# ai-decentralized/BloomBee

Hardware: AMD Instinct MI355X
Metric: decode tokens/sec, llama-3-8b greedy, pipeline over RCCL/xGMI (higher is better)
Workload: dtype bfloat16; 1 GPU; model=llama-3-8b, global_batch=32, seq_len=2048, parallelism=pp1, micro_batches=1

## Files before the change

bloombee_amd/models/llama/block.py:

```python
from __future__ import annotations

import math
from typing import Optional

import torch
import torch.nn.functional as F

from bloombee_amd import ops
from bloombee_amd.kv.paged import SessionHandle
from bloombee_amd.models.base import ModelConfig
from bloombee_amd.models.block_common import (
    FamilyBlock, RopeTables, pack_q4, paged_attention_qkv, rms_train,
    rope_attn_train, rotary_positions, split_heads, swiglu_mlp_train)


class LlamaBlock(FamilyBlock):
    def __init__(self, config: ModelConfig, layer_index: int = 0,
                 rope: Optional[RopeTables] = None):
        super().__init__(config, layer_index)
        H = config.hidden_size
        D = config.head_dim
        Hq, Hkv = config.num_attention_heads, config.num_key_value_heads
        I = config.intermediate_size
        self.Hq, self.Hkv, self.D, self.I = Hq, Hkv, D, I
        self.scale = 1.0 / math.sqrt(D)
        p = self.p
        self.input_norm_w = p(H)
        self.qkv_w = p((Hq + 2 * Hkv) * D, H)
        self.o_w = p(H, Hq * D)
        self.post_norm_w = p(H)
        self.gate_up_w = p(2 * I, H)
        self.down_w = p(H, I)
        self.rope = rope if rope is not None else RopeTables(config)
        self._ss_h2 = None
        self._ss_hidden = None
        self._ss_valid = False
        self._splitk_cnt = None

    def _fuse_norm_gate(self, hidden) -> bool:
        return (getattr(self, "_w4", None) is None
                and getattr(self, "lora_delta", None) is None
                and ops.fuse_norm_linear_ok(hidden, self.qkv_w)
                and self.I % 256 == 0 and (2 * self.I) % 64 == 0
                and (self.Hq * self.D) % 256 == 0
                and self.config.hidden_size % 64 == 0)

    def _ensure_ss_bufs(self, device) -> None:
        if self._ss_h2 is None or self._ss_h2.device != device:
            st = self.config.hidden_size // 64
            self._ss_h2 = torch.empty(st * 32, dtype=torch.float32,
                                      device=device)
            self._ss_hidden = torch.empty_like(self._ss_h2)
            self._splitk_cnt = torch.zeros(2 * st, dtype=torch.int32,
                                           device=device)

    @torch.no_grad()
    def fold_norm_weights(self):
        if getattr(self, "_norm_folded", False):
            return
        self._norm_fold_orig = (self.input_norm_w.detach().clone(),
                                self.post_norm_w.detach().clone())
        self.qkv_w.data = (self.qkv_w.float()
                           * self.input_norm_w.float()).to(self.qkv_w.dtype)
        self.gate_up_w.data = (self.gate_up_w.float()
                               * self.post_norm_w.float()).to(self.gate_up_w.dtype)
        self.input_norm_w.data.fill_(1.0)
        self.post_norm_w.data.fill_(1.0)
        self._norm_folded = True

    @torch.no_grad()
    def unfold_norm_weights(self):
        if not getattr(self, "_norm_folded", False):
            return
        inw, pnw = self._norm_fold_orig
        self.input_norm_w.data.copy_(inw)
        self.post_norm_w.data.copy_(pnw)
        den_i = inw.float().abs().clamp_min(1e-6) * inw.float().sign().where(
            inw.float() != 0, torch.ones_like(inw.float()))
        den_p = pnw.float().abs().clamp_min(1e-6) * pnw.float().sign().where(
            pnw.float() != 0, torch.ones_like(pnw.float()))
        self.qkv_w.data = (self.qkv_w.float() / den_i).to(self.qkv_w.dtype)
        self.gate_up_w.data = (self.gate_up_w.float() / den_p).to(self.gate_up_w.dtype)
        self._norm_folded = False

    @torch.no_grad()
    def quantize_weights_q4(self, keep_full: bool = False):
        pack_q4(self, ("qkv_w", "o_w", "gate_up_w", "down_w"), keep_full)
        return self

    def _lin(self, x, w, name, **kw):
        w4 = getattr(self, "_w4", None)
        if w4 is not None and name in w4:
            packed, scale, zero, N = w4[name]
            y = ops.linear_w4(x, packed, scale, zero, N, **kw)
        else:
            y = ops.linear(x, w, **kw)
        ld = getattr(self, "lora_delta", None)
        if ld is not None:
            d = ld(name, x)
            if d is not None:
                y = y + d
        return y

    def _post_qkv(self, qkv: torch.Tensor, B: int, T: int) -> torch.Tensor:
        return qkv

    def _post_qkv_train(self, q: torch.Tensor, k: torch.Tensor):
        return q, k

    @torch.no_grad()
    def forward_inference(
        self,
        hidden: torch.Tensor,
        kv: SessionHandle,
        start_pos: torch.Tensor,
        position_ids: Optional[torch.Tensor] = None,
        tree_mask: Optional[torch.Tensor] = None,
    ) -> torch.Tensor:
        B, T, H = hidden.shape
        Hq, Hkv, D = self.Hq, self.Hkv, self.D
        cfg = self.config

        fuse_norm = self._fuse_norm_gate(hidden)
        self._ss_valid = False
        if fuse_norm and not getattr(self, "_norm_folded", False):
            self.fold_norm_weights()
        pb = getattr(self, "prev_block", None)
        defer = (fuse_norm and type(self)._post_qkv is LlamaBlock._post_qkv
                 and ops.fuse_qkv_rope_ok(hidden, self.qkv_w, D))
        if fuse_norm and pb is not None and getattr(pb, "_ss_valid", False):
            qkv = ops.linear(hidden, self.qkv_w,
                             norm=(None, cfg.rms_norm_eps),
                             ss_in=pb._ss_hidden, defer_combine=defer)
        elif defer:
            x = ops.rms_norm(hidden, self.input_norm_w, cfg.rms_norm_eps)
            qkv = ops.linear(x, self.qkv_w, defer_combine=True)
        else:
            x = ops.rms_norm(hidden, self.input_norm_w, cfg.rms_norm_eps)
            qkv = self._lin(x, self.qkv_w, "qkv_w")
        if not defer:
            qkv = self._post_qkv(qkv, B, T)
        cos, sin = self.rope.get(hidden.device)
        kp = kv.k_pages(self.layer_index)
        vp = kv.v_pages(self.layer_index)
        pt = kv.page_table()
        position_ids = rotary_positions(kv, start_pos, position_ids, T)
        ctx_lens = None
        if defer and qkv.dtype == torch.float32:
            qkv, ctx_lens = ops.rope_kv_write_part(
                qkv, None, B, T, Hq, Hkv, cos, sin, position_ids, kp, vp, pt,
                start_pos)
        else:
            ops.rope_kv_write_(qkv, Hq, Hkv, cos, sin, position_ids, kp, vp,
                               pt, start_pos)
        attn = paged_attention_qkv(qkv, kv, self.layer_index, start_pos, Hq,
                                   Hkv, self.scale, tree_mask=tree_mask,
                                   ctx_lens=ctx_lens)
        if fuse_norm:
            self._ensure_ss_bufs(hidden.device)
            st = H // 64
            h2 = ops.linear(attn, self.o_w, residual=hidden,
                            ss_out=self._ss_h2,
                            cnt=(self._splitk_cnt[:st]
                                 if ops.inlaunch_combine_ok(attn, self.o_w, "o")
                                 else None))
            act = ops.linear_swiglu(h2, self.gate_up_w,
                                    norm=(None, cfg.rms_norm_eps),
                                    ss_in=self._ss_h2)
            out = ops.linear(act, self.down_w, residual=h2,
                             ss_out=self._ss_hidden,
                             cnt=(self._splitk_cnt[st:]
                                  if ops.inlaunch_combine_ok(act, self.down_w,
                                                             "down")
                                  else None))
            self._ss_valid = True
            return out
        a = self._lin(attn, self.o_w, "o_w")

        h2, y = ops.rms_norm_residual(a, hidden, self.post_norm_w, cfg.rms_norm_eps)
        return self._lin(ops.swiglu(self._lin(y, self.gate_up_w, "gate_up_w")),
                         self.down_w, "down_w", residual=h2)

    def forward_train(self, hidden: torch.Tensor, start_pos: int = 0) -> torch.Tensor:
        eps = self.config.rms_norm_eps

        def lin(x_, w, name):
            y = F.linear(x_, w)
            ld = getattr(self, "lora_delta", None)
            if ld is not None:
                d = ld(name, x_)
                if d is not None:
                    y = y + d
            return y

        x = rms_train(hidden, self.input_norm_w, eps)
        q, k, v = split_heads(lin(x, self.qkv_w, "qkv_w"), self.Hq, self.Hkv,
                              self.D)
        q, k = self._post_qkv_train(q, k)
        attn = rope_attn_train(q, k, v, self.rope, start_pos, self.scale)
        h2 = hidden + lin(attn, self.o_w, "o_w")
        y = rms_train(h2, self.post_norm_w, eps)
        return h2 + swiglu_mlp_train(y, self.gate_up_w, self.down_w)
```

bloombee_amd/ops/__init__.py:

```python
from bloombee_amd.ops.interface import (
    HAVE_HIP_OPS,
    alibi_slopes_for,
    attn_decode,
    attn_paged,
    attn_paged_mixed,
    attn_paged_mixed_qkv,
    attn_paged_qkv,
    attn_prefill,
    attn_train,
    fuse_norm_linear_ok,
    fuse_qkv_rope_ok,
    fuse_swiglu_ok,
    gelu_tanh,
    hip_ops,
    inlaunch_combine_ok,
    kv_gather,
    kv_write,
    layer_norm,
    linear,
    linear_swiglu,
    linear_w4,
    mfma_selftest,
    moe_gemm_grouped,
    moe_gemm_grouped_w4,
    quant4_pack,
    quant4_unpack,
    rms_norm,
    rms_norm_residual,
    rope_apply_,
    rope_kv_write_,
    rope_kv_write_part,
    rope_cos_sin,
    set_attn_sparsity,
    swiglu,
)
```

bloombee_amd/ops/hip/common.h:

```cpp
#pragma once

#include <hip/hip_runtime.h>

#define DEVINL __device__ __forceinline__

typedef __attribute__((ext_vector_type(8))) short short8;
typedef __attribute__((ext_vector_type(4))) short short4v;
typedef __attribute__((ext_vector_type(4))) float f32x4;
typedef __attribute__((ext_vector_type(2))) float f32x2;

static constexpr int WAVE = 64;
static constexpr float LOG2E = 1.4426950408889634f;
static constexpr float NEG_BIG = -1e30f;

typedef __attribute__((ext_vector_type(8))) __bf16 bf16x8;
DEVINL bf16x8 as_bf16x8(short8 s) { return __builtin_bit_cast(bf16x8, s); }

DEVINL float bf2f(unsigned short u) {
  union { unsigned int i; float f; } v;
  v.i = ((unsigned int)u) << 16;
  return v.f;
}

DEVINL unsigned short f2bf(float f) {
// ... 19 lines not shown
  *reinterpret_cast<short8*>(p) = v;
}

DEVINL float wave_reduce_sum(float x) {
#pragma unroll
  for (int m = 1; m < WAVE; m <<= 1) x += __shfl_xor(x, m);
  return x;
}

DEVINL float wave_reduce_max(float x) {
#pragma unroll
  for (int m = 1; m < WAVE; m <<= 1) x = fmaxf(x, __shfl_xor(x, m));
  return x;
}

DEVINL float group16_reduce_sum(float x) {
#pragma unroll
  for (int m = 1; m < 16; m <<= 1) x += __shfl_xor(x, m);
  return x;
}

DEVINL float group16_reduce_max(float x) {
#pragma unroll
  for (int m = 1; m < 16; m <<= 1) x = fmaxf(x, __shfl_xor(x, m));
  return x;
}

DEVINL float fast_exp2(float x) { return __builtin_amdgcn_exp2f(x); }

DEVINL float fast_expf(float x) { return __builtin_amdgcn_exp2f(x * LOG2E); }

DEVINL long ldiv_up(long a, long b) { return (a + b - 1) / b; }

#define HIP_OK(expr)                                                         \
  do {                                                                       \
    hipError_t _e = (expr);                                                  \
    if (_e != hipSuccess) {                                                  \
      TORCH_CHECK(false, "HIP error: ", hipGetErrorString(_e), " at ",       \
                  __FILE__, ":", __LINE__);                                  \
    }                                                                        \
  } while (0)
```

bloombee_amd/ops/hip/ext.hip:

```cpp

#include <torch/extension.h>
#include <c10/hip/HIPStream.h>
#include <hip/hip_runtime.h>
#include <cstdlib>

#include "common.h"

#include "elementwise.hip"
#include "kvcache.hip"
#include "attn_decode.hip"
#include "attn_decode_mfma.hip"
#include "attn_sparse.hip"
#include "attn_prefill.hip"
#include "attn_train.hip"
#include "gemm_skinny.hip"
#include "moe_gemm.hip"
#include "w4_gemm.hip"
#include "moe_gemm_w4.hip"
#include "mfma_selftest.hip"
#include "quant4.hip"
#include "wire.h"

typedef __attribute__((ext_vector_type(8))) short short8_h;

// ... 129 lines not shown
  int ksplit = (int)ksplit_req;
  if (ksplit <= 0) {
    static const int ks_big = [] {
      const char* e = std::getenv("BBAMD_GEMM_KSPLIT_BIG");
      return e ? std::atoi(e) : 1;
    }();
    if (N / 64 >= 256) ksplit = ks_big;
    else ksplit = (int)std::min<long>(K / 512,
                                      std::max<long>(1, std::min<long>(8, 1024 / (N / 64))));
    ksplit = std::max(1, ksplit);
  }
  if (K % 256 != 0)
    return {ksplit, (int)((K / 32 + ksplit - 1) / ksplit) * 32, false};
  const SplitK s = split_k_chunks((int)K, 256, ksplit);
  return {s.ksplit, s.kchunk, true};
}

static constexpr int kWringDepths[] = {2, 4};

static int skinny_wring(long req) {
  static const int env = [] {
    const char* e = std::getenv("BBAMD_GEMM_WRING");
    return e ? std::atoi(e) : 0;
  }();
  if (req <= 0) req = env;
  if (req <= 0) return 2;
  TORCH_CHECK(std::find(std::begin(kWringDepths), std::end(kWringDepths), req) !=
                  std::end(kWringDepths),
              "gemm_skinny W ring depth must be 2 or 4, got ", req);
  return (int)req;
}

template <int MT, int EPI, typename... Args>
static void launch_skinny_v2(int depth, dim3 grid, Args... args) {
  if (depth == 2)
    gemm_skinny_v2_kernel<MT, EPI><<<grid, 256, 0, cur_stream()>>>(args...);
  else
    gemm_skinny_v2_ring_kernel<MT, EPI, 4><<<grid, 256, 0, cur_stream()>>>(args...);
}

struct W4Plan {
  bool gemv;
  int ksplit, kchunk;
};

static W4Plan w4_plan(long M, long N, long K, long ksplit_req) {
  TORCH_CHECK(N >= 64 && K >= 128 && K % 128 == 0 && N % 64 == 0,
              "K%128, N%64 required");
  if (M == 1 && K % 2048 == 0 && K / 2048 <= 7) return {true, 1, (int)K};
  int ksplit = (int)ksplit_req;
  if (ksplit <= 0) {
    ksplit = (int)std::max<long>(1, std::min<long>(K / 512, 1792 / (N / 64)));
  }
  const SplitK s = split_k_chunks((int)K, 128, ksplit);
  return {false, s.ksplit, s.kchunk};
}

static SplitK moe_w4_plan(long E, long N, long K, long S, long ksplit_req) {
  TORCH_CHECK(N >= 64 && K >= 128 && K % 128 == 0 && N % 64 == 0,
              "K%128, N%64 required");
  int ksplit = (int)ksplit_req;
  if (ksplit <= 0) {
    const long blocks = (N / 64) * std::max<long>(1, std::min<long>(E, S));
    ksplit = (int)std::max<long>(1, std::min<long>(K / 512, 1792 / blocks));
  }
  return split_k_chunks((int)K, 128, ksplit);
}
// ... 836 lines not shown
  dim3 grid(N / 64, ksplit);
  dispatch_mtile(M, [&](auto mt) {
    gemm_skinny_w4_kernel<decltype(mt)::value><<<grid, 256, 0, cur_stream()>>>(
        ap, qp, scp, zp, ksplit == 1 ? rp : nullptr, ksplit == 1 ? bp : nullptr,
        cp, part.p, M, N, K, plan.kchunk, ksplit);
  });
  if (ksplit > 1) {
    const long total = (long)M * N;
    const int cgrid = (int)std::min<long>((total + 255) / 256, 2048);
    gemm_skinny_combine_kernel<<<cgrid, 256, 0, cur_stream()>>>(
        part.p, rp, bp, cp, M, N, ksplit);
  }
  return C;
}


static const float* ss_in_operand(const Operands& ops,
                                  const c10::optional<torch::Tensor>& ss_in,
                                  int* nstripes) {
  *nstripes = 0;
  if (!ss_in.has_value()) return nullptr;
  TORCH_CHECK(ss_in->numel() % 32 == 0, "ss_in must be f32 (nstripes,32)");
  *nstripes = (int)(ss_in->numel() / 32);
  return ops.ptr<F32>(*ss_in, "ss_in");
}

torch::Tensor gemm_skinny(torch::Tensor A, torch::Tensor W,
                          c10::optional<torch::Tensor> residual,
                          c10::optional<torch::Tensor> bias, long ksplit_req,
                          c10::optional<torch::Tensor> norm_w, double eps,
                          c10::optional<torch::Tensor> ss_in,
                          c10::optional<torch::Tensor> ss_out,
                          long norm_mode_req, bool defer_combine,
                          c10::optional<torch::Tensor> cnt, long wring_req) {
  Operands ops(A, "A");
  const auto* ap = ops.ptr<Bf16>(A, "A");
  const auto* wp = ops.ptr<Bf16>(W, "W");
  const int K = A.size(-1);
  const int M = A.numel() / K;
  const int N = W.size(0);
  TORCH_CHECK(M <= 32, "gemm_skinny is for M <= 32, got ", M);
  TORCH_CHECK(W.size(1) == K, "A/W K mismatch");
  TORCH_CHECK(K % 32 == 0 && N % 64 == 0, "K%32, N%64 required");
  int norm_mode = (int)norm_mode_req;
  const auto* nwp = ops.ptr<Bf16>(norm_w, "norm_w", true, K);
  if (nwp && norm_mode == 0) norm_mode = 1;
  TORCH_CHECK(norm_mode != 1 || nwp, "norm_mode 1 needs norm_w");
  if (norm_mode)
    TORCH_CHECK(K % 256 == 0, "fused rmsnorm needs the v2 (K%256) kernel");
  TORCH_CHECK(!ss_in.has_value() || norm_mode != 0,
              "ss_in only meaningful with a norm mode");
  int nstripes = 0;
  const float* ssinp = ss_in_operand(ops, ss_in, &nstripes);
  float* ssoutp = ops.ptr<F32>(ss_out, "ss_out", true, (long)(N / 64) * 32);
  const auto* rp = ops.ptr<Bf16>(residual, "residual", true, (long)M * N);
  const auto* bp = ops.ptr<Bf16>(bias, "bias", true, N);
  int* cntp = ops.ptr<I32>(cnt, "cnt");
  auto sizes = A.sizes().vec();
  sizes.back() = N;
  auto C = torch::empty(sizes, A.options());
  auto* cp = ops.ptr<Bf16>(C, "C");
  const SkinnyPlan plan = skinny_plan(N, K, ksplit_req);
  const int ksplit = plan.ksplit, kchunk = plan.kchunk;
  const Slabs part = alloc_slabs(ops, A, ksplit, M, N);
  const int wring =
      !plan.v2 ? 0
      : norm_mode == 1
          ? 2
          : skinny_wring(wring_req);
  if (cnt.has_value() && ksplit > 1 && plan.v2) {
    TORCH_CHECK(!defer_combine, "cnt and defer_combine exclude each other");
    TORCH_CHECK(cnt->numel() >= N / 64, "cnt must be int32 of >= N/64 entries");
    dispatch_mtile(M, [&](auto mt) {
      launch_skinny_v2<decltype(mt)::value, 2>(
          wring, dim3((N / 64) * ksplit), ap, wp, rp, bp, cp, part.p, M, N, K,
          kchunk, ksplit, nwp, (float)eps, norm_mode, ssinp, nstripes, ssoutp,
          cntp);
    });
    return C;
  }
  dim3 grid(N / 64, ksplit);
  dispatch_mtile(M, [&](auto mt) {
    if (plan.v2)
      launch_skinny_v2<decltype(mt)::value, 0>(
          wring, grid, ap, wp, ksplit == 1 ? rp : nullptr,
          ksplit == 1 ? bp : nullptr, cp, part.p, M, N, K, kchunk, ksplit, nwp,
          (float)eps, norm_mode, ssinp, nstripes,
          ksplit == 1 ? ssoutp : nullptr, (int*)nullptr);
    else {
      TORCH_CHECK(!norm_mode && (!ssoutp || ksplit > 1),
                  "fused norm / ss_out need the v2 (K%256) kernel");
      gemm_skinny_kernel<decltype(mt)::value><<<grid, 256, 0, cur_stream()>>>(
          ap, wp, ksplit == 1 ? rp : nullptr, ksplit == 1 ? bp : nullptr, cp,
          part.p, M, N, K, ksplit);
    }
  });
  if (ksplit > 1 && defer_combine) {
    TORCH_CHECK(!rp && !ssoutp, "defer_combine takes no residual / ss_out");
    return part.t;
  }
  if (ksplit > 1) {
    if (ssoutp || (N % 64 == 0 && N / 64 >= 64)) {
      dim3 cg(N / 64, (M + 15) / 16);
      gemm_skinny_combine_ss_kernel<<<cg, 256, 0, cur_stream()>>>(
          part.p, rp, bp, cp, ssoutp, M, N, ksplit);
    } else {
      const long total = (long)M * N;
      const int cgrid = (int)std::min<long>((total + 255) / 256, 2048);
      gemm_skinny_combine_kernel<<<cgrid, 256, 0, cur_stream()>>>(
          part.p, rp, bp, cp, M, N, ksplit);
    }
  }
  return C;
}

torch::Tensor gemm_skinny_swiglu(torch::Tensor A, torch::Tensor W, double eps,
                                 c10::optional<torch::Tensor> ss_in,
                                 long norm_mode_req, long wring_req) {
  Operands ops(A, "A");
  const auto* ap = ops.ptr<Bf16>(A, "A");
  const auto* wp = ops.ptr<Bf16>(W, "W");
  const int K = A.size(-1);
  const int M = A.numel() / K;
  const int N = W.size(0);
  const int I = N / 2;
  const int norm_mode = (int)norm_mode_req;
  TORCH_CHECK(M >= 1 && M <= 32, "gemm_skinny_swiglu is for 1 <= M <= 32, got ", M);
  TORCH_CHECK(W.dim() == 2 && W.size(1) == K, "A/W K mismatch");
  TORCH_CHECK(N % 2 == 0 && I % 32 == 0 && K % 256 == 0,
              "gemm_skinny_swiglu needs I % 32 == 0 and K % 256 == 0");
  TORCH_CHECK(norm_mode == 0 || norm_mode == 2, "norm_mode must be 0 or 2");
  TORCH_CHECK(!ss_in.has_value() || norm_mode == 2,
              "ss_in only meaningful with norm_mode 2");
  int nstripes = 0;
  const float* ssinp = ss_in_operand(ops, ss_in, &nstripes);
  auto sizes = A.sizes().vec();
  sizes.back() = I;
  auto C = torch::empty(sizes, A.options());
  auto* cp = ops.ptr<Bf16>(C, "C");
  const int wring = skinny_wring(wring_req);
  dispatch_mtile(M, [&](auto mt) {
    launch_skinny_v2<decltype(mt)::value, 1>(
        wring, dim3(I / 32), ap, wp, (const unsigned short*)nullptr,
        (const unsigned short*)nullptr, cp, (float*)nullptr, M, N, K, K, 1,
        (const unsigned short*)nullptr, (float)eps, norm_mode, ssinp, nstripes,
        (float*)nullptr, (int*)nullptr);
  });
  return C;
}


std::vector<torch::Tensor> quant4_pack(torch::Tensor x) {
  Operands ops(x, "x");
  const auto* xp = ops.ptr<Bf16>(x, "x");
  const long ncols = x.size(-1);
  TORCH_CHECK(ncols % 64 == 0, "quant4 needs cols % 64 == 0");
  const long nrows = x.numel() / ncols;
  auto packed = torch::empty({nrows, ncols / 2}, x.options().dtype(at::kByte));
  auto scale = torch::empty({nrows, ncols / 64}, x.options().dtype(at::kHalf));
  auto zero = torch::empty_like(scale);
  const long ngroups = nrows * (ncols / 64);
  if (ngroups == 0) return {packed, scale, zero};
  const int wpb = 4;
  quant4_pack_kernel<64><<<(ngroups + wpb - 1) / wpb, wpb * 64, 0, cur_stream()>>>(
      xp, ops.ptr<U8>(packed, "packed"), ops.ptr<F16>(scale, "scale"),
      ops.ptr<F16>(zero, "zero"), nrows, ncols);
  return {packed, scale, zero};
}

torch::Tensor quant4_unpack(torch::Tensor packed, torch::Tensor scale,
                            torch::Tensor zero) {
  Operands ops(packed, "packed");
  auto* qp = ops.ptr<U8>(packed, "packed");
  TORCH_CHECK(packed.dim() == 2, "packed must be (rows, cols/2)");
  const long nrows = packed.size(0), ncols = packed.size(1) * 2;
  TORCH_CHECK(ncols % 64 == 0, "quant4 needs cols % 64 == 0");
// ... 38 lines not shown
  return C;
}

PYBIND11_MODULE(TORCH_EXTENSION_NAME, m) {
  m.def("rms_norm", &rms_norm);
  m.def("rms_norm_residual", &rms_norm_residual);
  m.def("layer_norm", &layer_norm);
  m.def("rope_apply_", &rope_apply_);
  m.def("swiglu", &swiglu);
  m.def("gelu_tanh", &gelu_tanh);
  m.def("add_bf16", &add_bf16);
  m.def("kv_write", &kv_write);
  m.def("kv_gather", &kv_gather);
  m.def("wire_deflate", &wire_deflate);
  m.def("wire_inflate", &wire_inflate);
  m.def("wire_deflate_mt", &wire_deflate_mt);
  m.def("wire_inflate_mt", &wire_inflate_mt);
  m.def("attn_decode", &attn_decode);
  m.def("attn_decode_qkv", &attn_decode_qkv);
  m.def("attn_decode_mixed", &attn_decode_mixed);
  m.def("attn_decode_sparse", &attn_decode_sparse);
  m.def("attn_decode_sparse_qkv", &attn_decode_sparse_qkv);
  m.def("attn_prefill_qkv", &attn_prefill_qkv);
  m.def("rope_kv_write_", &rope_kv_write_);
  m.def("attn_prefill", &attn_prefill);
  m.def("attn_train_fwd", &attn_train_fwd);
  m.def("attn_train_bwd", &attn_train_bwd);
  m.def("gemm_skinny", &gemm_skinny, py::arg("A"), py::arg("W"),
        py::arg("residual") = c10::nullopt, py::arg("bias") = c10::nullopt,
        py::arg("ksplit") = 0, py::arg("norm_w") = c10::nullopt,
        py::arg("eps") = 0.0, py::arg("ss_in") = c10::nullopt,
        py::arg("ss_out") = c10::nullopt, py::arg("norm_mode") = 0,
        py::arg("defer_combine") = false, py::arg("cnt") = c10::nullopt,
        py::arg("wring") = 0);
  m.def("gemm_skinny_swiglu", &gemm_skinny_swiglu, py::arg("A"), py::arg("W"),
        py::arg("eps") = 0.0, py::arg("ss_in") = c10::nullopt,
        py::arg("norm_mode") = 0, py::arg("wring") = 0);
  m.def("gemm_skinny_plan", &gemm_skinny_plan);
  m.def("gemm_skinny_wring_plan", &gemm_skinny_wring_plan, py::arg("N"),
        py::arg("K"), py::arg("ksplit") = 0, py::arg("wring") = 0);
  m.def("rope_kv_write_part", &rope_kv_write_part);
  m.def("moe_gemm", &moe_gemm);
  m.def("gemm_w4", &gemm_w4);
  m.def("gemm_w4_plan", &gemm_w4_plan);
  m.def("moe_gemm_w4", &moe_gemm_w4);
  m.def("moe_gemm_w4_plan", &moe_gemm_w4_plan);
  m.def("quant4_pack", &quant4_pack);
  m.def("quant4_unpack", &quant4_unpack);
  m.def("mfma_selftest", &mfma_selftest);
  m.def("kv_stream_probe", &kv_stream_probe);
}
```

bloombee_amd/ops/hip/gemm_skinny.hip:

```cpp

#include "common.h"

template <int MT>
__global__ __launch_bounds__(256) void gemm_skinny_kernel(
    const unsigned short* __restrict__ A,
    const unsigned short* __restrict__ W,
    const unsigned short* __restrict__ R,
    const unsigned short* __restrict__ bias,
    unsigned short* __restrict__ C,
    float* __restrict__ Cpart,
    int M, int N, int K, int ksplit) {
  const int wave = threadIdx.x / WAVE;
  const int lane = threadIdx.x & (WAVE - 1);
  const int li = lane & 15;
  const int hi = lane >> 4;
  const int n0 = blockIdx.x * 64 + wave * 16;
  if (n0 >= N) return;
  const int split = blockIdx.y;
  const int kchunk = ((K / 32 + ksplit - 1) / ksplit) * 32;
  const int k0 = split * kchunk;
  const int k1 = min(K, k0 + kchunk);

  const unsigned short* wrow = W + (long)(n0 + li) * K;
  int arow[MT];
// ... 71 lines not shown
#pragma unroll
    for (int e = 0; e < 4; ++e) v[e] += p[e];
  }
#pragma unroll
  for (int e = 0; e < 4; ++e) {
    if (bias) v[e] += bf2f(bias[n0 + c4 + e]);
    if (R) v[e] += bf2f(R[i + e]);
  }
  short4v o4;
#pragma unroll
  for (int e = 0; e < 4; ++e) o4[e] = (short)f2bf(v[e]);
  *reinterpret_cast<short4v*>(C + i) = o4;
  if (ssout) {
    float vs = v[0] * v[0] + v[1] * v[1] + v[2] * v[2] + v[3] * v[3];
#pragma unroll
    for (int msk = 1; msk < 16; msk <<= 1) vs += __shfl_xor(vs, msk);
    if ((lane & 15) == 0) ssout[(long)stripe * 32 + m] = vs;
  }
}

template <int I>
struct WringIdx {
  static constexpr int value = I;
};

template <int DEPTH, int N, typename F>
DEVINL void wring_tail_dispatch(int nrem, F& f) {
  if constexpr (N <= 2 * DEPTH - 2) {
    if (nrem == N) f(WringIdx<N>{});
    else wring_tail_dispatch<DEPTH, N + 2>(nrem, f);
  }
}

template <int MT, int EPI, int DEPTH>
DEVINL void gemm_skinny_v2_body(
    const unsigned short* __restrict__ A,
    const unsigned short* __restrict__ W,
    const unsigned short* __restrict__ R,
    const unsigned short* __restrict__ bias,
    unsigned short* __restrict__ C,
    float* __restrict__ Cpart,
    int M, int N, int K, int kchunk, int ksplit,
    const unsigned short* __restrict__ nw,
    float eps, int norm_mode,
    const float* __restrict__ ssin,
    int nstripes,
    float* __restrict__ ssout,
    int* cnt) {
  static_assert(DEPTH == 2 || DEPTH % 4 == 0, "ring: whole waves per A row");
  constexpr int U = 4;
  constexpr int KSTEP = DEPTH * 128;
  constexpr int RSTRIDE = KSTEP + 8;
  constexpr int RPIECE = KSTEP / 8;
  constexpr int NPIECE = (32 * KSTEP) / (256 * 8);
  __shared__ __attribute__((aligned(16))) unsigned short atile[32 * RSTRIDE];
  __shared__ float ssp[256];
  __shared__ float invr[32];

  const int wave = threadIdx.x / WAVE;
  const int lane = threadIdx.x & (WAVE - 1);
  const int li = lane & 15;
  const int hi = lane >> 4;
  int tile = blockIdx.x;
  {
    const int nwg = gridDim.x;
    const int xcd = tile % 8, orig8 = tile / 8;
    const int q = nwg / 8, r = nwg % 8;
    if (nwg >= 8)
      tile = (xcd < r ? xcd * (q + 1) : r * (q + 1) + (xcd - r) * q) + orig8;
  }
  int split = blockIdx.y;
  if constexpr (EPI == 2) {
    split = tile % ksplit;
    tile /= ksplit;
  }
  const int n0 = tile * 64 + wave * 16;
  const int k0 = split * kchunk;
  const int k1 = min(K, k0 + kchunk);

  const unsigned short* wrow = W + (long)(n0 + li) * K;
  if constexpr (EPI == 1)
    wrow = W + ((long)(li < 8 ? 0 : N / 2 - 8) + tile * 32 + wave * 8 + li) * K;

  f32x4 acc[MT];
#pragma unroll
  for (int t = 0; t < MT; ++t) acc[t] = (f32x4){0.f, 0.f, 0.f, 0.f};

  short8 aregs[NPIECE];
  short8 nregs[DEPTH == 2 ? NPIECE : 1];
  const int wave_s = __builtin_amdgcn_readfirstlane(wave);
  auto load_a = [&](int ks, int lim = 1 << 30) {
#pragma unroll
    for (int j = 0; j < NPIECE; ++j) {
      if constexpr (DEPTH == 2) {
        const int flat = threadIdx.x + j * 256;
        const int row = min(flat / RPIECE, M - 1);
        const int off = (flat % RPIECE) * 8;
        aregs[j] = *reinterpret_cast<const short8*>(A + (long)row * K + ks + off);
        if (norm_mode == 1)
          nregs[j] = *reinterpret_cast<const short8*>(nw + ks + off);
      } else {
        const int fw = wave_s + j * 4;
        const int row = min(fw / (RPIECE / 64), M - 1);
        const unsigned off =
            min((fw % (RPIECE / 64)) * 64 + lane, lim / 8 - 1) * 16u;
        aregs[j] = *reinterpret_cast<const short8*>(
            reinterpret_cast<const char*>(A + (long)row * K + ks) + off);
      }
    }
  };
  auto store_a = [&]() {
#pragma unroll
    for (int j = 0; j < NPIECE; ++j) {
      const int flat = threadIdx.x + j * 256;
      short8 v = aregs[j];
      if (DEPTH == 2 && norm_mode == 1) {
        const float ir = invr[flat / RPIECE >= M ? M - 1 : flat / RPIECE];
#pragma unroll
        for (int e = 0; e < 8; ++e)
          v[e] = (short)f2bf(bf2f((unsigned short)v[e]) * ir *
                             bf2f((unsigned short)nregs[j][e]));
      }
      *reinterpret_cast<short8*>(atile + (flat / RPIECE) * RSTRIDE +
                                 (flat % RPIECE) * 8) = v;
    }
  };

  bf16x8 bB0[U], bB1[U];
  auto issue0 = [&](int k) {
#pragma unroll
    for (int u = 0; u < U; ++u)
      bB0[u] = as_bf16x8(
          *reinterpret_cast<const short8*>(wrow + k + u * 32 + hi * 8));
  };
  auto issue1 = [&](int k) {
#pragma unroll
    for (int u = 0; u < U; ++u)
      bB1[u] = as_bf16x8(
          *reinterpret_cast<const short8*>(wrow + k + u * 32 + hi * 8));
  };
  auto mfma_set = [&](bf16x8* bB, int half) {
#pragma unroll
    for (int u = 0; u < U; ++u)
#pragma unroll
      for (int t = 0; t < MT; ++t) {
        bf16x8 afrag = as_bf16x8(*reinterpret_cast<const short8*>(
            atile + (t * 16 + li) * RSTRIDE + half * 128 + u * 32 + hi * 8));
        acc[t] = __builtin_amdgcn_mfma_f32_16x16x32_bf16(afrag, bB[u], acc[t],
                                                         0, 0, 0);
      }
  };

  auto reduce_invr = [&]() {
    if (ssin) {
      const int row = threadIdx.x & 31, grp = threadIdx.x >> 5;
      float s0 = 0.f, s1 = 0.f, s2 = 0.f, s3 = 0.f;
      int s = grp;
      for (; s + 24 < nstripes; s += 32) {
        s0 += ssin[(long)s * 32 + row];
        s1 += ssin[(long)(s + 8) * 32 + row];
        s2 += ssin[(long)(s + 16) * 32 + row];
        s3 += ssin[(long)(s + 24) * 32 + row];
      }
      for (; s < nstripes; s += 8) s0 += ssin[(long)s * 32 + row];
      ssp[threadIdx.x] = (s0 + s1) + (s2 + s3);
      __syncthreads();
      if (threadIdx.x < 32) {
        float t = 0.f;
#pragma unroll
        for (int g = 0; g < 8; ++g) t += ssp[g * 32 + threadIdx.x];
        invr[threadIdx.x] = rsqrtf(t / K + eps);
      }
// ... 223 lines not shown
      __syncthreads();
      if (threadIdx.x < 32)
        ssout[(long)tile * 32 + threadIdx.x] =
            ssp[threadIdx.x] + ssp[32 + threadIdx.x] +
            ssp[64 + threadIdx.x] + ssp[96 + threadIdx.x];
    }
  } else {
    float* dst = Cpart + (long)split * M * N;
#pragma unroll
    for (int t = 0; t < MT; ++t)
#pragma unroll
      for (int reg = 0; reg < 4; ++reg) {
        const int m = t * 16 + hi * 4 + reg;
        if (m >= M) continue;
        float v = acc[t][reg];
        if (norm_mode == 2) v *= invr[m];
        dst[(long)m * N + n0 + li] = v;
      }
  }
}

#define SKINNY_V2_PARAMS                                                      \
  const unsigned short *__restrict__ A, const unsigned short *__restrict__ W, \
      const unsigned short *__restrict__ R,                                   \
      const unsigned short *__restrict__ bias, unsigned short *__restrict__ C, \
      float *__restrict__ Cpart, int M, int N, int K, int kchunk, int ksplit, \
      const unsigned short *__restrict__ nw, float eps, int norm_mode,        \
      const float *__restrict__ ssin, int nstripes, float *__restrict__ ssout, \
      int *cnt
#define SKINNY_V2_ARGS                                                       \
  A, W, R, bias, C, Cpart, M, N, K, kchunk, ksplit, nw, eps, norm_mode, ssin, \
      nstripes, ssout, cnt

template <int MT, int EPI = 0>
__global__ __launch_bounds__(256) void gemm_skinny_v2_kernel(SKINNY_V2_PARAMS) {
  gemm_skinny_v2_body<MT, EPI, 2>(SKINNY_V2_ARGS);
}

template <int MT, int EPI, int DEPTH>
__global__ __launch_bounds__(256, 3) void gemm_skinny_v2_ring_kernel(
    SKINNY_V2_PARAMS) {
  gemm_skinny_v2_body<MT, EPI, DEPTH>(SKINNY_V2_ARGS);
}

__global__ __launch_bounds__(256) void gemm_skinny_combine_ss_kernel(
    const float* __restrict__ Cpart, const unsigned short* __restrict__ R,
    const unsigned short* __restrict__ bias, unsigned short* __restrict__ C,
    float* __restrict__ ssout, int M, int N, int ksplit) {
  const int lane = threadIdx.x & (WAVE - 1);
  const int m = blockIdx.y * 16 + (threadIdx.x >> 6) * 4 + (lane >> 4);
  if (m >= M) return;
  gemm_skinny_combine_lane(Cpart, R, bias, C, ssout, M, N, ksplit, blockIdx.x,
                           m, lane);
}

__global__ void gemm_skinny_combine_kernel(
    const float* __restrict__ Cpart, const unsigned short* __restrict__ R,
    const unsigned short* __restrict__ bias, unsigned short* __restrict__ C,
    int M, int N, int ksplit) {
  const long total = (long)M * N;
  for (long i = blockIdx.x * (long)blockDim.x + threadIdx.x; i < total;
       i += (long)gridDim.x * blockDim.x) {
    float v = 0.f;
    for (int s = 0; s < ksplit; ++s) v += Cpart[(long)s * total + i];
    if (bias) v += bf2f(bias[i % N]);
    if (R) v += bf2f(R[i]);
    C[i] = f2bf(v);
  }
}
// ... 1 lines not shown
```

bloombee_amd/ops/interface.py:

```python
from __future__ import annotations

import importlib
import math
import os
from typing import Optional, Tuple

import torch

from bloombee_amd.ops import reference as ref
from bloombee_amd.ops.reference import alibi_slopes as alibi_slopes_for
from bloombee_amd.ops.reference import rope_cos_sin
from bloombee_amd.utils.logging import get_logger

logger = get_logger(__name__)

try:
    hip_ops = importlib.import_module("bloombee_amd.ops._hip_ops")
    HAVE_HIP_OPS = True
except ImportError as e:
    hip_ops = None
    HAVE_HIP_OPS = False
    _import_error = e


# ... 229 lines not shown
    if alibi_slopes is not None and not _on_gpu(q) and not sparse_decode:
        if scale is None:
            scale = 1.0 / math.sqrt(q.shape[-1])
        return ref.attn_paged(q, k_pages, v_pages, page_table, q_start, scale,
                              alibi_slopes=alibi_slopes,
                              sliding_window=_window_or_none(window))
    if tree_mask is not None:
        if scale is None:
            scale = 1.0 / math.sqrt(q.shape[-1])
        if (_on_gpu(q) and _TREE_KERNEL and window == 0
                and q.shape[-1] <= 256 and alibi_slopes is None):
            _require_ext()
            tm = tree_mask.to(q.device).contiguous().bool()
            return hip_ops.attn_prefill(q.contiguous(), k_pages, v_pages,
                                        page_table, q_start.int(), scale, 0,
                                        None, tm)
        return ref.attn_paged(q, k_pages, v_pages, page_table,
                              q_start.to(q.device), scale,
                              tree_mask=tree_mask.to(q.device))
    if Tq == 1:
        ctx_lens = q_start + 1
        return attn_decode(q, k_pages, v_pages, page_table, ctx_lens, scale,
                           window, alibi_slopes=alibi_slopes)
    return attn_prefill(q, k_pages, v_pages, page_table, q_start, scale, window,
                        alibi_slopes=alibi_slopes)


def linear(x: torch.Tensor, w: torch.Tensor, residual: Optional[torch.Tensor] = None,
           bias: Optional[torch.Tensor] = None,
           norm: Optional[tuple] = None,
           ss_in: Optional[torch.Tensor] = None,
           ss_out: Optional[torch.Tensor] = None,
           defer_combine: bool = False,
           cnt: Optional[torch.Tensor] = None) -> torch.Tensor:
    M = x.numel() // x.shape[-1]
    N, K = w.shape[0], x.shape[-1]
    if (_on_gpu(x) and M <= 32 and x.dtype == torch.bfloat16
            and K % 256 == 0 and N % 64 == 0):
        _require_ext()
        nw, eps, mode = None, 0.0, 0
        if norm is not None:
            eps = float(norm[1])
            if norm[0] is None:
                mode = 2
            else:
                nw = norm[0].contiguous()
                mode = 1
        return hip_ops.gemm_skinny(x.contiguous(), w, residual, bias,
                                   _INLAUNCH_KSPLIT if cnt is not None else 0,
                                   nw, eps, ss_in if norm is not None else None,
                                   ss_out, mode, defer_combine, cnt)
    if defer_combine or cnt is not None:
        raise RuntimeError("defer_combine / cnt require the GPU skinny-GEMM "
                           "path (callers gate on fuse_norm_linear_ok)")
    if norm is not None:
        nw = norm[0]
        if nw is None:
            nw = torch.ones(x.shape[-1], dtype=x.dtype, device=x.device)
        x = rms_norm(x, nw, norm[1])
    y = torch.nn.functional.linear(x, w, bias)
    if residual is not None:
        y = y + residual.view_as(y)
    if ss_out is not None:
        raise RuntimeError("ss_out requires the GPU skinny-GEMM path "
                           "(callers gate on fuse_norm_linear_ok)")
    return y


_FUSE_NORM = os.environ.get("BBAMD_FUSE_NORM", "1") != "0"


def fuse_norm_linear_ok(x: torch.Tensor, w: torch.Tensor) -> bool:
    K = x.shape[-1]
    return (_FUSE_NORM and _on_gpu(x) and x.numel() // K <= 32
            and x.dtype == torch.bfloat16 and K % 256 == 0
            and w.shape[0] % 64 == 0 and HAVE_HIP_OPS)


_FUSE_SWIGLU = os.environ.get("BBAMD_FUSE_SWIGLU", "1") != "0"
_FUSE_QKV_ROPE = os.environ.get("BBAMD_FUSE_QKV_ROPE", "1") != "0"
_INLAUNCH_DEFAULT = "0"


def _parse_inlaunch(v: str) -> frozenset:
    if v in ("", "0"):
        return frozenset()
    if v == "1":
        return frozenset(("o", "down"))
    return frozenset(x.strip() for x in v.split(",")) & {"o", "down"}


_INLAUNCH_COMBINE = _parse_inlaunch(
    os.environ.get("BBAMD_INLAUNCH_COMBINE", _INLAUNCH_DEFAULT))
_INLAUNCH_KSPLIT = int(os.environ.get("BBAMD_INLAUNCH_KSPLIT", "0"))


def fuse_swiglu_ok(x: torch.Tensor, gate_up_w: torch.Tensor) -> bool:
    N, K = gate_up_w.shape[0], x.shape[-1]
    return (_FUSE_SWIGLU and fuse_norm_linear_ok(x, gate_up_w)
            and hip_ops.gemm_skinny_plan(N, K, 0)[0] == 1)


def fuse_qkv_rope_ok(x: torch.Tensor, qkv_w: torch.Tensor, D: int) -> bool:
    return (_FUSE_QKV_ROPE and fuse_norm_linear_ok(x, qkv_w) and D % 8 == 0)


def inlaunch_combine_ok(x: torch.Tensor, w: torch.Tensor, which: str) -> bool:
    return which in _INLAUNCH_COMBINE and fuse_norm_linear_ok(x, w)


def linear_swiglu(x: torch.Tensor, gate_up_w: torch.Tensor,
                  norm: Optional[tuple] = None,
                  ss_in: Optional[torch.Tensor] = None) -> torch.Tensor:
    if fuse_swiglu_ok(x, gate_up_w):
        _require_ext()
        assert norm is None or norm[0] is None, \
            "linear_swiglu takes the folded-weight norm only"
        return hip_ops.gemm_skinny_swiglu(
            x.contiguous(), gate_up_w,
            float(norm[1]) if norm is not None else 0.0, ss_in,
            2 if norm is not None else 0)
    return swiglu(linear(x, gate_up_w, norm=norm, ss_in=ss_in))


_MIXED_KERNEL = os.environ.get("BBAMD_MIXED_KERNEL", "1") not in ("", "0")


def _mixed_kernel_ok(D: int) -> bool:
    return _MIXED_KERNEL and (D <= 256 or D == 512)


def _attn_mixed_gpu(q_or_qkv, q4, k_pages, v_pages, page_table, ctx_lens,
                    host_k, host_v, scale, window, alibi_slopes, n_split=0):
    _require_ext()
    B, Hq, _, D = q4.shape
    S_host = host_k.shape[2]
    dev = q4.device
    al = _alibi_on(alibi_slopes, dev)
    lo = 0
    if window > 0:
        lo = (S_host + ctx_lens.long().cpu() - window).clamp_(min=0)
        if int(lo.min()) >= S_host:
            if q_or_qkv.dim() == 3:
                return hip_ops.attn_decode_qkv(
                    q_or_qkv, Hq, k_pages, v_pages, page_table,
                    ctx_lens.int(), scale, window, n_split)
            return (hip_ops.attn_decode(q_or_qkv.contiguous(), k_pages,
                                        v_pages, page_table, ctx_lens.int(),
                                        scale, window, n_split, al)
                    .permute(0, 2, 1, 3).reshape(B, 1, Hq * D))
    ml, acc = ref.attn_host_partial(
        q4[:, :, 0].float().cpu(), host_k, host_v, scale, lo,
        alibi_slopes.cpu() if alibi_slopes is not None else None)
    n_ml = B * Hq * 2
    stage = torch.empty(n_ml + B * Hq * D, dtype=torch.float32,
# ... 181 lines not shown
```

bloombee_amd/ops/reference.py:

```python
from __future__ import annotations

import math
from typing import Optional, Tuple

import torch



def rms_norm(x: torch.Tensor, weight: torch.Tensor, eps: float = 1e-5) -> torch.Tensor:
    xf = x.float()
    var = xf.pow(2).mean(dim=-1, keepdim=True)
    y = xf * torch.rsqrt(var + eps)
    return (y * weight.float()).to(x.dtype)


def rms_norm_residual(
    x: torch.Tensor, residual: torch.Tensor, weight: torch.Tensor, eps: float = 1e-5
) -> Tuple[torch.Tensor, torch.Tensor]:
    h = (x.float() + residual.float()).to(x.dtype)
    return h, rms_norm(h, weight, eps)


def layer_norm(
    x: torch.Tensor, weight: torch.Tensor, bias: Optional[torch.Tensor], eps: float = 1e-5
# ... 310 lines not shown
        S = offs[-1]
    C = torch.zeros(S, N, dtype=A.dtype, device=A.device)
    for e in range(E):
        a, b = offs[e], offs[e + 1]
        if b <= a:
            continue
        slots = torch.arange(a, b, device=A.device)
        rows = rowmap[slots].long() if rowmap is not None else slots
        y = A[rows].float() @ W[e].float().t()
        if scale is not None:
            y = y * scale[slots].float().unsqueeze(1)
        C[slots] = y.to(A.dtype)
    return C


def moe_gemm_grouped_w4(A: torch.Tensor, packed: torch.Tensor,
                        scale: torch.Tensor, zero: torch.Tensor,
                        off: torch.Tensor,
                        rowmap: Optional[torch.Tensor] = None,
                        slot_scale: Optional[torch.Tensor] = None,
                        S: Optional[int] = None) -> torch.Tensor:
    E, N, Kh = packed.shape
    K = Kh * 2
    offs = off.tolist()
    W = torch.zeros(E, N, K, dtype=A.dtype, device=A.device)
    for e in range(E):
        if offs[e + 1] > offs[e]:
            W[e] = quant4_unpack(packed[e].reshape(N, K // 64, 32),
                                 scale[e].reshape(N, K // 64),
                                 zero[e].reshape(N, K // 64), A.dtype)
    return moe_gemm_grouped(A, W, off, rowmap, slot_scale, S)


def attn_train(q: torch.Tensor, k: torch.Tensor, v: torch.Tensor, scale: float,
               window: int = 0,
               alibi_slopes: Optional[torch.Tensor] = None) -> torch.Tensor:
    B, T, Hq, D = q.shape
    G = Hq // k.shape[2]
    q, k, v = (t.permute(0, 2, 1, 3) for t in (q, k, v))
    if G > 1:
        k = k.repeat_interleave(G, dim=1)
        v = v.repeat_interleave(G, dim=1)
    scores = torch.matmul(q.float(), k.float().transpose(-1, -2))
    if scale != 1.0:
        scores = scores * scale
    if alibi_slopes is not None:
        scores = scores + alibi_slopes.view(1, Hq, 1, 1).to(scores.device) * \
            torch.arange(T, dtype=torch.float32,
                         device=scores.device).view(1, 1, 1, T)
    mask = torch.ones(T, T, dtype=torch.bool, device=scores.device).tril()
    if window > 0:
        pos = torch.arange(T, device=scores.device)
        mask &= pos.view(1, T) > pos.view(T, 1) - window
    scores = scores.masked_fill(~mask, float("-inf"))
    p = torch.softmax(scores, dim=-1)
    out = torch.matmul(p, v.float()).to(q.dtype)
    return out.permute(0, 2, 1, 3)
```

Baseline: 5503 tokens/s.

## Pre-pack skinny GEMM weights into wave-contiguous tiles for decode

Adds a packed weight layout that groups 16 rows by 32-wide K blocks, so each wave's load of a K block reads one contiguous 512-element chunk. The skinny GEMM and SwiGLU kernels gain a PACKED template path that indexes this layout. LlamaBlock caches the packed copies, keyed on tensor pointer and version, and uses them for the Llama-3-8B shapes when enough free memory remains. It targets scattered row-strided weight loads in memory-bound decode GEMMs, at the cost of a second copy of every weight and extra invalidation logic.

New measurement: 5905 tokens/s (median of 6 runs). +7.3%, better.

```diff
diff --git a/bloombee_amd/models/llama/block.py b/bloombee_amd/models/llama/block.py
--- a/bloombee_amd/models/llama/block.py
+++ b/bloombee_amd/models/llama/block.py
@@ -1,6 +1,7 @@
 from __future__ import annotations
 
 import math
+import os
 from typing import Optional
 
 import torch
@@ -12,6 +13,21 @@
 from bloombee_amd.models.block_common import (
     FamilyBlock, RopeTables, pack_q4, paged_attention_qkv, rms_train,
     rope_attn_train, rotary_positions, split_heads, swiglu_mlp_train)
+
+
+_PACK_W_DEFAULT = "auto"
+_PACK_W_FASTER: frozenset = frozenset((
+    (6144, 4096),
+    (4096, 4096),
+    (28672, 4096),
+    (4096, 14336),
+))
+_PACK_W_RESERVE = 8
+
+
+def _pack_w_mode() -> str:
+    v = os.environ.get("BBAMD_PACK_W", _PACK_W_DEFAULT).strip().lower()
+    return v if v in ("0", "1") else "auto"
 
 
 class LlamaBlock(FamilyBlock):
@@ -36,6 +52,37 @@
         self._ss_hidden = None
         self._ss_valid = False
         self._splitk_cnt = None
+        self._wpacked = {}
+
+    def _drop_packed(self) -> None:
+        self._wpacked.clear()
+
+    def _packed(self, name: str, swiglu: bool = False):
+        mode = _pack_w_mode()
+        if mode == "0":
+            self._drop_packed()
+            return None
+        w = getattr(self, name)
+        ent = self._wpacked.get(name)
+        if ent is not None:
+            src, ver, wp = ent
+            if src.data_ptr() == w.data_ptr() and ver == w._version:
+                return wp
+            del self._wpacked[name]
+        if w.is_cuda and torch.cuda.is_current_stream_capturing():
+            return None
+        wp = None
+        if mode == "1" or self._pack_auto_ok(w):
+            wp = ops.pack_skinny_w(w.detach(), swiglu)
+        self._wpacked[name] = (w.detach(), w._version, wp)
+        return wp
+
+    @staticmethod
+    def _pack_auto_ok(w: torch.Tensor) -> bool:
+        if tuple(w.shape) not in _PACK_W_FASTER or not w.is_cuda:
+            return False
+        free, total = torch.cuda.mem_get_info(w.device)
+        return free - w.numel() * w.element_size() >= total // _PACK_W_RESERVE
 
     def _fuse_norm_gate(self, hidden) -> bool:
         return (getattr(self, "_w4", None) is None
@@ -58,6 +105,7 @@
     def fold_norm_weights(self):
         if getattr(self, "_norm_folded", False):
             return
+        self._drop_packed()
         self._norm_fold_orig = (self.input_norm_w.detach().clone(),
                                 self.post_norm_w.detach().clone())
         self.qkv_w.data = (self.qkv_w.float()
@@ -72,6 +120,7 @@
     def unfold_norm_weights(self):
         if not getattr(self, "_norm_folded", False):
             return
+        self._drop_packed()
         inw, pnw = self._norm_fold_orig
         self.input_norm_w.data.copy_(inw)
         self.post_norm_w.data.copy_(pnw)
@@ -85,6 +134,7 @@
 
     @torch.no_grad()
     def quantize_weights_q4(self, keep_full: bool = False):
+        self._drop_packed()
         pack_q4(self, ("qkv_w", "o_w", "gate_up_w", "down_w"), keep_full)
         return self
 
@@ -125,16 +175,21 @@
         self._ss_valid = False
         if fuse_norm and not getattr(self, "_norm_folded", False):
             self.fold_norm_weights()
+        if self._wpacked and (getattr(self, "_w4", None) is not None
+                              or getattr(self, "lora_delta", None) is not None):
+            self._drop_packed()
         pb = getattr(self, "prev_block", None)
         defer = (fuse_norm and type(self)._post_qkv is LlamaBlock._post_qkv
                  and ops.fuse_qkv_rope_ok(hidden, self.qkv_w, D))
         if fuse_norm and pb is not None and getattr(pb, "_ss_valid", False):
             qkv = ops.linear(hidden, self.qkv_w,
                              norm=(None, cfg.rms_norm_eps),
-                             ss_in=pb._ss_hidden, defer_combine=defer)
+                             ss_in=pb._ss_hidden, defer_combine=defer,
+                             w_packed=self._packed("qkv_w"))
         elif defer:
             x = ops.rms_norm(hidden, self.input_norm_w, cfg.rms_norm_eps)
-            qkv = ops.linear(x, self.qkv_w, defer_combine=True)
+            qkv = ops.linear(x, self.qkv_w, defer_combine=True,
+                             w_packed=self._packed("qkv_w"))
         else:
             x = ops.rms_norm(hidden, self.input_norm_w, cfg.rms_norm_eps)
             qkv = self._lin(x, self.qkv_w, "qkv_w")
@@ -163,16 +218,22 @@
                             ss_out=self._ss_h2,
                             cnt=(self._splitk_cnt[:st]
                                  if ops.inlaunch_combine_ok(attn, self.o_w, "o")
-                                 else None))
+                                 else None),
+                            w_packed=self._packed("o_w"))
             act = ops.linear_swiglu(h2, self.gate_up_w,
                                     norm=(None, cfg.rms_norm_eps),
-                                    ss_in=self._ss_h2)
+                                    ss_in=self._ss_h2,
+                                    w_packed=(self._packed("gate_up_w", True)
+                                              if ops.fuse_swiglu_ok(
+                                                  h2, self.gate_up_w)
+                                              else None))
             out = ops.linear(act, self.down_w, residual=h2,
                              ss_out=self._ss_hidden,
                              cnt=(self._splitk_cnt[st:]
                                   if ops.inlaunch_combine_ok(act, self.down_w,
                                                              "down")
-                                  else None))
+                                  else None),
+                             w_packed=self._packed("down_w"))
             self._ss_valid = True
             return out
         a = self._lin(attn, self.o_w, "o_w")
diff --git a/bloombee_amd/ops/__init__.py b/bloombee_amd/ops/__init__.py
--- a/bloombee_amd/ops/__init__.py
+++ b/bloombee_amd/ops/__init__.py
@@ -23,6 +23,7 @@
     mfma_selftest,
     moe_gemm_grouped,
     moe_gemm_grouped_w4,
+    pack_skinny_w,
     quant4_pack,
     quant4_unpack,
     rms_norm,
diff --git a/bloombee_amd/ops/hip/common.h b/bloombee_amd/ops/hip/common.h
--- a/bloombee_amd/ops/hip/common.h
+++ b/bloombee_amd/ops/hip/common.h
@@ -75,6 +75,11 @@
 
 DEVINL long ldiv_up(long a, long b) { return (a + b - 1) / b; }
 
+static constexpr int SKINNY_PACK_BLOCK = 512;
+__host__ __device__ inline long skinny_packed_offset(int g, int kb, int K) {
+  return ((long)g * (K / 32) + kb) * SKINNY_PACK_BLOCK;
+}
+
 #define HIP_OK(expr)                                                         \
   do {                                                                       \
     hipError_t _e = (expr);                                                  \
diff --git a/bloombee_amd/ops/hip/ext.hip b/bloombee_amd/ops/hip/ext.hip
--- a/bloombee_amd/ops/hip/ext.hip
+++ b/bloombee_amd/ops/hip/ext.hip
@@ -185,7 +185,15 @@
 }
 
 template <int MT, int EPI, typename... Args>
-static void launch_skinny_v2(int depth, dim3 grid, Args... args) {
+static void launch_skinny_v2(int depth, bool packed, dim3 grid, Args... args) {
+  if constexpr (EPI != 2) {
+    if (packed) {
+      TORCH_CHECK(depth == 2, "packed W runs at ring depth 2 only");
+      gemm_skinny_v2_kernel<MT, EPI, true><<<grid, 256, 0, cur_stream()>>>(args...);
+      return;
+    }
+  }
+  TORCH_CHECK(!packed, "packed W: plain and SwiGLU epilogues only");
   if (depth == 2)
     gemm_skinny_v2_kernel<MT, EPI><<<grid, 256, 0, cur_stream()>>>(args...);
   else
@@ -1088,7 +1096,8 @@
                           c10::optional<torch::Tensor> ss_in,
                           c10::optional<torch::Tensor> ss_out,
                           long norm_mode_req, bool defer_combine,
-                          c10::optional<torch::Tensor> cnt, long wring_req) {
+                          c10::optional<torch::Tensor> cnt, long wring_req,
+                          c10::optional<torch::Tensor> w_packed) {
   Operands ops(A, "A");
   const auto* ap = ops.ptr<Bf16>(A, "A");
   const auto* wp = ops.ptr<Bf16>(W, "W");
@@ -1124,22 +1133,25 @@
       : norm_mode == 1
           ? 2
           : skinny_wring(wring_req);
+  const auto* wpp = ops.ptr<Bf16>(w_packed, "w_packed", true, (long)N * K);
   if (cnt.has_value() && ksplit > 1 && plan.v2) {
     TORCH_CHECK(!defer_combine, "cnt and defer_combine exclude each other");
     TORCH_CHECK(cnt->numel() >= N / 64, "cnt must be int32 of >= N/64 entries");
     dispatch_mtile(M, [&](auto mt) {
       launch_skinny_v2<decltype(mt)::value, 2>(
-          wring, dim3((N / 64) * ksplit), ap, wp, rp, bp, cp, part.p, M, N, K,
-          kchunk, ksplit, nwp, (float)eps, norm_mode, ssinp, nstripes, ssoutp,
-          cntp);
+          wring, false, dim3((N / 64) * ksplit), ap, wp, rp, bp, cp, part.p, M,
+          N, K, kchunk, ksplit, nwp, (float)eps, norm_mode, ssinp, nstripes,
+          ssoutp, cntp);
     });
     return C;
   }
   dim3 grid(N / 64, ksplit);
+  const bool packed = wpp && wring == 2;
   dispatch_mtile(M, [&](auto mt) {
     if (plan.v2)
       launch_skinny_v2<decltype(mt)::value, 0>(
-          wring, grid, ap, wp, ksplit == 1 ? rp : nullptr,
+          wring, packed, grid, ap, packed ? wpp : wp,
+          ksplit == 1 ? rp : nullptr,
           ksplit == 1 ? bp : nullptr, cp, part.p, M, N, K, kchunk, ksplit, nwp,
           (float)eps, norm_mode, ssinp, nstripes,
           ksplit == 1 ? ssoutp : nullptr, (int*)nullptr);
@@ -1172,7 +1184,8 @@
 
 torch::Tensor gemm_skinny_swiglu(torch::Tensor A, torch::Tensor W, double eps,
                                  c10::optional<torch::Tensor> ss_in,
-                                 long norm_mode_req, long wring_req) {
+                                 long norm_mode_req, long wring_req,
+                                 c10::optional<torch::Tensor> w_packed) {
   Operands ops(A, "A");
   const auto* ap = ops.ptr<Bf16>(A, "A");
   const auto* wp = ops.ptr<Bf16>(W, "W");
@@ -1195,9 +1208,12 @@
   auto C = torch::empty(sizes, A.options());
   auto* cp = ops.ptr<Bf16>(C, "C");
   const int wring = skinny_wring(wring_req);
+  const auto* wpp = ops.ptr<Bf16>(w_packed, "w_packed", true, (long)N * K);
+  const bool packed = wpp && wring == 2;
   dispatch_mtile(M, [&](auto mt) {
     launch_skinny_v2<decltype(mt)::value, 1>(
-        wring, dim3(I / 32), ap, wp, (const unsigned short*)nullptr,
+        wring, packed, dim3(I / 32), ap, packed ? wpp : wp,
+        (const unsigned short*)nullptr,
         (const unsigned short*)nullptr, cp, (float*)nullptr, M, N, K, K, 1,
         (const unsigned short*)nullptr, (float)eps, norm_mode, ssinp, nstripes,
         (float*)nullptr, (int*)nullptr);
@@ -1302,10 +1318,11 @@
         py::arg("eps") = 0.0, py::arg("ss_in") = c10::nullopt,
         py::arg("ss_out") = c10::nullopt, py::arg("norm_mode") = 0,
         py::arg("defer_combine") = false, py::arg("cnt") = c10::nullopt,
-        py::arg("wring") = 0);
+        py::arg("wring") = 0, py::arg("w_packed") = c10::nullopt);
   m.def("gemm_skinny_swiglu", &gemm_skinny_swiglu, py::arg("A"), py::arg("W"),
         py::arg("eps") = 0.0, py::arg("ss_in") = c10::nullopt,
-        py::arg("norm_mode") = 0, py::arg("wring") = 0);
+        py::arg("norm_mode") = 0, py::arg("wring") = 0,
+        py::arg("w_packed") = c10::nullopt);
   m.def("gemm_skinny_plan", &gemm_skinny_plan);
   m.def("gemm_skinny_wring_plan", &gemm_skinny_wring_plan, py::arg("N"),
         py::arg("K"), py::arg("ksplit") = 0, py::arg("wring") = 0);
diff --git a/bloombee_amd/ops/hip/gemm_skinny.hip b/bloombee_amd/ops/hip/gemm_skinny.hip
--- a/bloombee_amd/ops/hip/gemm_skinny.hip
+++ b/bloombee_amd/ops/hip/gemm_skinny.hip
@@ -127,7 +127,7 @@
   }
 }
 
-template <int MT, int EPI, int DEPTH>
+template <int MT, int EPI, int DEPTH, bool PACKED = false>
 DEVINL void gemm_skinny_v2_body(
     const unsigned short* __restrict__ A,
     const unsigned short* __restrict__ W,
@@ -143,6 +143,8 @@
     float* __restrict__ ssout,
     int* cnt) {
   static_assert(DEPTH == 2 || DEPTH % 4 == 0, "ring: whole waves per A row");
+  static_assert(!PACKED || (DEPTH == 2 && EPI != 2),
+                "packed W: depth 2, plain and SwiGLU epilogues only");
   constexpr int U = 4;
   constexpr int KSTEP = DEPTH * 128;
   constexpr int RSTRIDE = KSTEP + 8;
@@ -176,6 +178,10 @@
   const unsigned short* wrow = W + (long)(n0 + li) * K;
   if constexpr (EPI == 1)
     wrow = W + ((long)(li < 8 ? 0 : N / 2 - 8) + tile * 32 + wave * 8 + li) * K;
+  if constexpr (PACKED)
+    wrow = W + skinny_packed_offset(
+                   tile * 4 + __builtin_amdgcn_readfirstlane(wave), 0, K) +
+           lane * 8;
 
   f32x4 acc[MT];
 #pragma unroll
@@ -222,17 +228,21 @@
   };
 
   bf16x8 bB0[U], bB1[U];
+  auto wptr = [&](int k, int u) -> const unsigned short* {
+    if constexpr (PACKED) return wrow + (k / 32 + u) * SKINNY_PACK_BLOCK;
+    else return wrow + k + u * 32 + hi * 8;
+  };
   auto issue0 = [&](int k) {
 #pragma unroll
     for (int u = 0; u < U; ++u)
       bB0[u] = as_bf16x8(
-          *reinterpret_cast<const short8*>(wrow + k + u * 32 + hi * 8));
+          *reinterpret_cast<const short8*>(wptr(k, u)));
   };
   auto issue1 = [&](int k) {
 #pragma unroll
     for (int u = 0; u < U; ++u)
       bB1[u] = as_bf16x8(
-          *reinterpret_cast<const short8*>(wrow + k + u * 32 + hi * 8));
+          *reinterpret_cast<const short8*>(wptr(k, u)));
   };
   auto mfma_set = [&](bf16x8* bB, int half) {
 #pragma unroll
@@ -522,9 +532,9 @@
   A, W, R, bias, C, Cpart, M, N, K, kchunk, ksplit, nw, eps, norm_mode, ssin, \
       nstripes, ssout, cnt
 
-template <int MT, int EPI = 0>
+template <int MT, int EPI = 0, bool PACKED = false>
 __global__ __launch_bounds__(256) void gemm_skinny_v2_kernel(SKINNY_V2_PARAMS) {
-  gemm_skinny_v2_body<MT, EPI, 2>(SKINNY_V2_ARGS);
+  gemm_skinny_v2_body<MT, EPI, 2, PACKED>(SKINNY_V2_ARGS);
 }
 
 template <int MT, int EPI, int DEPTH>
diff --git a/bloombee_amd/ops/interface.py b/bloombee_amd/ops/interface.py
--- a/bloombee_amd/ops/interface.py
+++ b/bloombee_amd/ops/interface.py
@@ -285,7 +285,8 @@
            ss_in: Optional[torch.Tensor] = None,
            ss_out: Optional[torch.Tensor] = None,
            defer_combine: bool = False,
-           cnt: Optional[torch.Tensor] = None) -> torch.Tensor:
+           cnt: Optional[torch.Tensor] = None,
+           w_packed: Optional[torch.Tensor] = None) -> torch.Tensor:
     M = x.numel() // x.shape[-1]
     N, K = w.shape[0], x.shape[-1]
     if (_on_gpu(x) and M <= 32 and x.dtype == torch.bfloat16
@@ -302,7 +303,8 @@
         return hip_ops.gemm_skinny(x.contiguous(), w, residual, bias,
                                    _INLAUNCH_KSPLIT if cnt is not None else 0,
                                    nw, eps, ss_in if norm is not None else None,
-                                   ss_out, mode, defer_combine, cnt)
+                                   ss_out, mode, defer_combine, cnt, 0,
+                                   w_packed)
     if defer_combine or cnt is not None:
         raise RuntimeError("defer_combine / cnt require the GPU skinny-GEMM "
                            "path (callers gate on fuse_norm_linear_ok)")
@@ -364,7 +366,8 @@
 
 def linear_swiglu(x: torch.Tensor, gate_up_w: torch.Tensor,
                   norm: Optional[tuple] = None,
-                  ss_in: Optional[torch.Tensor] = None) -> torch.Tensor:
+                  ss_in: Optional[torch.Tensor] = None,
+                  w_packed: Optional[torch.Tensor] = None) -> torch.Tensor:
     if fuse_swiglu_ok(x, gate_up_w):
         _require_ext()
         assert norm is None or norm[0] is None, \
@@ -372,8 +375,12 @@
         return hip_ops.gemm_skinny_swiglu(
             x.contiguous(), gate_up_w,
             float(norm[1]) if norm is not None else 0.0, ss_in,
-            2 if norm is not None else 0)
+            2 if norm is not None else 0, 0, w_packed)
     return swiglu(linear(x, gate_up_w, norm=norm, ss_in=ss_in))
+
+
+def pack_skinny_w(w: torch.Tensor, swiglu: bool = False) -> torch.Tensor:
+    return ref.pack_skinny_w(w, swiglu)
 
 
 _MIXED_KERNEL = os.environ.get("BBAMD_MIXED_KERNEL", "1") not in ("", "0")
diff --git a/bloombee_amd/ops/reference.py b/bloombee_amd/ops/reference.py
--- a/bloombee_amd/ops/reference.py
+++ b/bloombee_amd/ops/reference.py
@@ -366,6 +366,35 @@
     return moe_gemm_grouped(A, W, off, rowmap, slot_scale, S)
 
 
+def skinny_rowmap(N: int, swiglu: bool = False,
+                  device=None) -> torch.Tensor:
+    p = torch.arange(N, device=device)
+    if not swiglu:
+        return p
+    g, li = p // 16, p % 16
+    return torch.where(li < 8, g * 8 + li, N // 2 + g * 8 + li - 8)
+
+
+def pack_skinny_w(w: torch.Tensor, swiglu: bool = False) -> torch.Tensor:
+    N, K = w.shape
+    assert N % 16 == 0 and K % 32 == 0, "packed skinny W needs N%16, K%32"
+    assert not swiglu or N % 64 == 0, "SwiGLU row map needs I % 32 == 0"
+    rows = w[skinny_rowmap(N, True, w.device)] if swiglu else w
+    return (rows.reshape(N // 16, 16, K // 32, 4, 8)
+            .permute(0, 2, 3, 1, 4).contiguous())
+
+
+def unpack_skinny_w(wp: torch.Tensor, swiglu: bool = False) -> torch.Tensor:
+    G, KB = wp.shape[0], wp.shape[1]
+    N, K = G * 16, KB * 32
+    rows = wp.permute(0, 3, 1, 2, 4).reshape(N, K)
+    if not swiglu:
+        return rows.contiguous()
+    w = torch.empty_like(rows)
+    w[skinny_rowmap(N, True, wp.device)] = rows
+    return w
+
+
 def attn_train(q: torch.Tensor, k: torch.Tensor, v: torch.Tensor, scale: float,
                window: int = 0,
                alibi_slopes: Optional[torch.Tensor] = None) -> torch.Tensor:
```
